# qiutang98/chord

Hardware: AMD Instinct MI355X
Metric: Gtri/s into 4K 64-bit visbuffer (higher is better)
Workload: dtype f32+u64; 1 GPU; street_4k_hzb; scene_triangles_lod0=2799616, objects=352, hzb=True, cull=flat, parallelism=single

## Files before the change

### chord_amd/csrc/chordvis_abi.cpp

```cpp

#include "device_layer.h"

#include <algorithm>
#include <cmath>
#include <cstddef>
#include <cstdio>
#include <cstring>

using namespace chord;

namespace chord {

int fail(ChordCtx* ctx, int code, const char* what, hipError_t e)
{
    if (ctx) {
        char buf[512];
        if (e != hipSuccess) std::snprintf(buf, sizeof(buf), "%s: %s (%d)", what, hipGetErrorString(e), (int)e);
        else std::snprintf(buf, sizeof(buf), "%s", what);
        ctx->lastError = buf;
    }
    return code;
}

}
// ... 1360 lines not shown
    CHORD_HIP(c, hipMemcpy(c->hzb[slot].minTexels, hostMin, sizeof(uint16_t) * c->hzb[slot].desc.totalTexels, hipMemcpyHostToDevice));
    c->hzb[slot].valid = true;
    c->hzb[slot].uploaded = true;
    c->historySlot = slot;
    return CHORDVIS_OK;
}

int chordvis_set_debug(ChordCtx* c, uint32_t flags)
{
    if (c) c->orderAge = c->orderAge1 = 0xFFFFFFFFu;

    if (!c) return CHORDVIS_E_INVALID;
    if (!RASTER_PROFILE && (flags & CHORD_DEBUG_PROFILE_BITS))
        return fail(c, CHORDVIS_E_INVALID, "set_debug: the phase clocks (bits 16, 512) need a library built with -DRASTER_PROFILE=1 (chord_amd/build.py --tag prof -DRASTER_PROFILE=1)");
    if (!RASTER_ABLATION && (flags & CHORD_DEBUG_ABLATION_BITS))
        return fail(c, CHORDVIS_E_INVALID, "set_debug: the ablation switches need a library built with -DRASTER_ABLATION=1 (chord_amd/build.py --tag abl -DRASTER_ABLATION=1)");
    c->debugFlags = flags;
    if (c->depthCtx) c->depthCtx->debugFlags = flags;
    return CHORDVIS_OK;
}

int chordvis_debug_tile_profile(ChordCtx* c, int pass, uint64_t* hostTicks, uint32_t* hostCounts, uint32_t capacity)
{
    if (!c || pass < 0 || pass > 1 || !hostTicks || !hostCounts || capacity < c->tilesX * c->tilesY) return fail(c, CHORDVIS_E_INVALID, "debug_tile_profile: bad arguments");
    CHORD_HIP(c, hipStreamSynchronize(c->stream));
    const size_t n = (size_t)c->tilesX * c->tilesY;
    CHORD_HIP(c, hipMemcpy(hostTicks, c->dTileClocks + (size_t)pass * CHORD_MAX_TILES, n * 8, hipMemcpyDeviceToHost));
    CHORD_HIP(c, hipMemcpy2D(hostCounts, 4, c->dFrameState->tileCount + (size_t)pass * c->tilesX * c->tilesY * CHORD_TILECOUNT_STRIDE, 4 * CHORD_TILECOUNT_STRIDE, 4, n, hipMemcpyDeviceToHost));
    if (capacity >= 9 * n)
        CHORD_HIP(c, hipMemcpy(hostTicks + n, c->dTileClocks + (size_t)2 * CHORD_MAX_TILES + (size_t)pass * CHORD_MAX_TILES * 8, n * 64, hipMemcpyDeviceToHost));
    return CHORDVIS_OK;
}

int chordvis_debug_graph_frames(ChordCtx* c, uint32_t pairs, float* msPerFrameStream, float* msPerFrameGraph)
{
    if (!c || !pairs || !msPerFrameStream || !msPerFrameGraph) return fail(c, CHORDVIS_E_INVALID, "debug_graph_frames: bad arguments");
    if (!c->ownStream) return fail(c, CHORDVIS_E_INVALID, "debug_graph_frames: needs a context-owned (capturable) stream");
    int rc;
    struct KeepOff { ChordCtx* c; uint32_t keep; ~KeepOff() { c->orderKeepFrames = keep; c->orderAge = c->orderAge1 = 0xFFFFFFFFu; } } keepOff{c, c->orderKeepFrames};
    c->orderKeepFrames = 0u;
    for (int i = 0; i < 4; i++) if ((rc = chordvis_render_frame(c))) return rc;
    hipEvent_t e0, e1;
    CHORD_HIP(c, hipEventCreate(&e0)); CHORD_HIP(c, hipEventCreate(&e1));
    CHORD_HIP(c, hipStreamSynchronize(c->stream));
    CHORD_HIP(c, hipEventRecord(e0, c->stream));
    for (uint32_t i = 0; i < 2 * pairs; i++) if ((rc = chordvis_render_frame(c))) return rc;
    CHORD_HIP(c, hipEventRecord(e1, c->stream));
    CHORD_HIP(c, hipEventSynchronize(e1));
    float ms = 0;
    CHORD_HIP(c, hipEventElapsedTime(&ms, e0, e1));
    *msPerFrameStream = ms / (2.0f * pairs);
    hipGraph_t graph; hipGraphExec_t exec;
    CHORD_HIP(c, hipStreamBeginCapture(c->stream, hipStreamCaptureModeRelaxed));
    rc = chordvis_render_frame(c);
    if (!rc) rc = chordvis_render_frame(c);
    hipError_t ce = hipStreamEndCapture(c->stream, &graph);
    if (rc) return rc;
    CHORD_HIP(c, ce);
    CHORD_HIP(c, hipGraphInstantiate(&exec, graph, nullptr, nullptr, 0));
    for (int i = 0; i < 4; i++) CHORD_HIP(c, hipGraphLaunch(exec, c->stream));
    CHORD_HIP(c, hipStreamSynchronize(c->stream));
    CHORD_HIP(c, hipEventRecord(e0, c->stream));
    for (uint32_t i = 0; i < pairs; i++) CHORD_HIP(c, hipGraphLaunch(exec, c->stream));
    CHORD_HIP(c, hipEventRecord(e1, c->stream));
    CHORD_HIP(c, hipEventSynchronize(e1));
    CHORD_HIP(c, hipEventElapsedTime(&ms, e0, e1));
// ... 143 lines not shown
```

### chord_amd/csrc/device_layer.h

```cpp
#pragma once

#include <hip/hip_runtime.h>
#include <cstddef>

#include <string>
#include <vector>

#include "chordvis.h"

#ifndef RASTER_PROFILE
#define RASTER_PROFILE 0
#endif
#ifndef RASTER_ABLATION
#define RASTER_ABLATION 0
#endif
#define CHORD_DEBUG_PROFILE_BITS (16u | 512u)
#define CHORD_DEBUG_ABLATION_BITS (1u | 2u | 32u | 64u | 128u | 256u | 1024u | 2048u | 4096u | 8192u | 16384u | 1048576u | 2097152u)

namespace chord {


struct DPrim {
    float    posMin[3]; uint32_t meshletBase;
    float    posMax[3]; uint32_t groupBase;
// ... 325 lines not shown
    uint32_t* dTileBins = nullptr;
    uint32_t* dBinPool = nullptr;
    unsigned long long* dBinChunkTab = nullptr;
    uint32_t binPoolChunks = 0;
    uint32_t binMaxChunks = CHORD_BIN_MAX_CHUNKS_DEFAULT;
    uint64_t limitRecords = 64ull << 20;
    uint32_t limitPoolChunks = 32768;
    uint32_t rasterSerial = 0;
    bool inFrame = false;
    uint32_t binCap = 0, tilesX = 0, tilesY = 0;
    chord::ClipTri* dClipTris = nullptr;
    uint32_t clipTriCap = 0;
    bool resolveFrame = false;
    bool resolveStale = false;
    uint32_t* dTileMarker = nullptr;
    uint32_t* dShadingTiles = nullptr;
    uint32_t* dTileOrder = nullptr;
    uint32_t* dTileOrderKeep = nullptr;
    uint32_t orderAge = 0xFFFFFFFFu;
    uint32_t* dTileOrderKeep1 = nullptr;
    uint32_t orderAge1 = 0xFFFFFFFFu;
    uint32_t orderFlip[2] = {0u, 0u};
    uint32_t orderKeepFrames = 1u;
    unsigned long long* dTileSlabs = nullptr;
    uint32_t tileItemCap = 0;
    uint32_t* dLargeList = nullptr;
    uint32_t largeCap = 0;
    chord::DeviceCounters* dCounters = nullptr;
    bool pendingClear = false;
    bool depthOnly = false, depthClamp = false;
    float depthBiasConst = 0.0f, depthBiasSlope = 0.0f;

    uint64_t launchCount = 0;
    uint64_t frameLaunchBase = 0;
    uint32_t lastFrameLaunches = 0;
    int timers = 0;
    std::vector<hipEvent_t> evPool;
    std::vector<int> stampTags;
    uint32_t framesStamped = 0;
    uint32_t timerPeriod = 1;
    uint32_t frameIndex = 0;
    bool stampThisFrame = false;
    uint32_t rasterCalls = 0;
    bool shouldStage1 = false;
    chord::CmdList lastRejected;
    bool hzbTailInCull = false;
    bool fuseCullFrame = false;
    const chord::HzbBuffers* fuseCullHzb = nullptr;
    bool fusedCullDone = false;
    uint32_t cullSerial = 0;
    unsigned long long* dCullLookback = nullptr;
    uint32_t debugFlags = 0;
    unsigned long long* dTileClocks = nullptr;
};

#define CHORD_LAUNCH(ctx, ...) do { (ctx)->launchCount++; hipLaunchKernelGGL(__VA_ARGS__); } while (0)

namespace chord {

int fail(ChordCtx* ctx, int code, const char* what, hipError_t e = hipSuccess);
int alloc_scene_work_buffers(ChordCtx* c);

#define CHORD_HIP(ctx, call)                                                         \
    do {                                                                             \
        hipError_t e_ = (call);                                                      \
        if (e_ != hipSuccess) return ::chord::fail((ctx), CHORDVIS_E_HIP, #call, e_); \
// ... 32 lines not shown
```

### chord_amd/csrc/kernels_raster.hip

```cpp

#include "device_layer.h"
#include "device_math.h"

#include <algorithm>
#include <cstdlib>
#include <cstring>
#include <type_traits>

namespace chord {

#define GUARD_BAND 1024.0f
#define LDS_VERTS 256
#define TILE CHORD_TILE
#define TILE_SHIFT CHORD_TILE_SHIFT
#define TPITCH (TILE + 1)
#define SMALL_AREA 256
#define TC_STRIDE CHORD_TILECOUNT_STRIDE
#define TC_BLOCKS 1u
#define TC_TICKET 2u
#ifndef CHORD_MASKED_FUSED
#define CHORD_MASKED_FUSED 1
#endif
#define TC_MASKED 3u

// ... 15 lines not shown
    unsigned long long* binChunkTab; uint32_t binStamp; uint32_t binMaxChunks;
    unsigned long long* blockPool; uint32_t blockCap;
    uint32_t blockForce;
    ClipTri* clipTris; uint32_t clipTriCap; uint32_t pass;
    uint32_t* largeList; uint32_t largeCap;
    uint32_t binInSetup;
    DeviceCounters* counters;
    uint2* tileOrder;
    unsigned long long* tileSlabs;
    uint32_t hzbFused;
    ChordHZBDesc hzbDesc;
    uint16_t* hzbMinA;
    uint16_t* hzbMinB; uint16_t* hzbMaxB;
    uint16_t* hzbExA;
    uint16_t* hzbExB;
    uint32_t* tileRange;
    unsigned long long* tileClocks;
    unsigned long long* tilePhase;
    uint32_t depthOnly, depthClamp;
    float biasConst, biasSlope;
    uint32_t clearTiles;
    uint32_t* binHint;
    uint32_t* countHint;
    uint32_t slotHot;
    uint32_t* hotTiles;
    uint32_t tileSlots;
    uint32_t tileSplitMin, tileSliceLen;
    uint2* tileOrderNext;
    uint32_t orderAll;
    uint32_t orderKept;
    uint32_t* heavyHint;
    uint32_t* tileTouched;
    uint32_t debug;
};
#define ABL(p, flag) (RASTER_ABLATION && ((p).debug & (flag)) != 0u)
#define DBG_NO_PIXELS   1u
#define DBG_NO_BIN      2u
#define DBG_TILE_CLOCKS 16u
#define DBG_NO_OUT      128u
#define DBG_NO_HZB      256u
#define DBG_SETUP_CLOCKS 512u
#define DBG_NO_VIS_STORE 1024u
#define DBG_NO_SPLIT    2048u
#define DBG_NO_TINY     32u
#define DBG_TILE_EXIT   64u
#define DBG_NO_ENTRY    8192u
#define DBG_NO_BATCH    16384u
#define DBG_NO_UNITS    4096u
#define DBG_SKIP_LIGHT  1048576u
#define DBG_SKIP_HEAVY  2097152u

template <typename T>
__device__ __forceinline__ T scalar_load(const T* ptr)
{
    return *reinterpret_cast<const __attribute__((address_space(4))) T*>(reinterpret_cast<uintptr_t>(ptr));
}
__device__ __forceinline__ const RasterParams* kernel_args()
{
    unsigned long long kp = (unsigned long long)__builtin_amdgcn_kernarg_segment_ptr();
    asm volatile("" : "+s"(kp));
    return reinterpret_cast<const RasterParams*>(kp);
}

__device__ __forceinline__ uint32_t mbcnt64(unsigned long long m) { return __builtin_amdgcn_mbcnt_hi((uint32_t)(m >> 32), __builtin_amdgcn_mbcnt_lo((uint32_t)m, 0u)); }
__device__ __forceinline__ int32_t bcast(int32_t v, int src) { return __builtin_amdgcn_readlane(v, src); }
__device__ __forceinline__ uint32_t bcast(uint32_t v, int src) { return (uint32_t)__builtin_amdgcn_readlane((int)v, src); }
// ... 1400 lines not shown
#undef SPHASE
}

__device__ __forceinline__ bool launch_is_dense(const RasterParams& p, uint32_t count)
{
    const unsigned long long pixels = (unsigned long long)p.Wi * (unsigned long long)p.Hi / (p.shard.ranks > 1u ? p.shard.ranks : 1u);
    return p.blockCap != 0u && p.leftCmds != nullptr && (p.blockForce != 0u || (unsigned long long)count * 16ull >= pixels);
}

#ifndef SETUP_MIN_WAVES
#define SETUP_MIN_WAVES 5
#endif
#ifndef BLOCKS_MIN_WAVES
#define BLOCKS_MIN_WAVES 6
#endif
#ifndef SETUP_MASKED_WAVES
#define SETUP_MASKED_WAVES 4
#endif
template <bool MASKED>
__global__ __launch_bounds__(256, MASKED ? SETUP_MASKED_WAVES : SETUP_MIN_WAVES) void raster_setup_kernel(RasterParams p)
{
    __shared__ __attribute__((aligned(16))) float sVert[6][4][LDS_VERTS];
    __shared__ uint32_t sClip[4][1 + CLIP_RANGES];
    const uint32_t c0 = __builtin_amdgcn_readfirstlane(min(blockIdx.x * 4u + (threadIdx.x >> 6), p.cmdCap - 1u));
    const uint32_t* __restrict__ cw = reinterpret_cast<const uint32_t*>(p.cmds + c0);
    const uint32_t f0 = scalar_load(cw), f1 = scalar_load(cw + 1), f2 = scalar_load(cw + 2);
    uint32_t count = *p.count;
    const ChordDrawCmd* cmds = p.cmds;
    bool firstValid = true;
    if (launch_is_dense(p, count)) { count = *p.leftCount; cmds = p.leftCmds; firstValid = false; }
    raster_setup_body<MASKED>(p, cmds, count, sVert, sClip[threadIdx.x >> 6], f0, f1, f2, firstValid);
}

template <bool HOT>
__global__ __launch_bounds__(256, BLOCKS_MIN_WAVES) void raster_setup_blocks_kernel(RasterParams p)
{
    __shared__ float sVert[6][4][BLOCKS_LDS_VERTS];
    __shared__ int32_t sSnap[2][4][BLOCKS_LDS_VERTS];
    __shared__ unsigned long long sWin[4][WIN * WIN];
    __shared__ SlotCache sSlots[HOT ? 4 : 1];
    const uint32_t count = *p.count;
    if (!launch_is_dense(p, count)) return;
    raster_setup_blocks_body<HOT>(p, count, sVert, sSnap, sWin, sSlots);
}

__device__ void raster_clip_part(const RasterParams& p, uint32_t block, uint32_t blocks)
{
    __shared__ float4 sPoly[2 * CLIP_MAXV * CLIP_THREADS];
    __shared__ float sPU[2 * CLIP_MAXV * CLIP_THREADS], sPV[2 * CLIP_MAXV * CLIP_THREADS];
    __shared__ int32_t sPX[CLIP_MAXV * CLIP_THREADS], sPY[CLIP_MAXV * CLIP_THREADS];
    __shared__ float sPD[CLIP_MAXV * CLIP_THREADS];
    if (threadIdx.x >= CLIP_THREADS) return;
    const ClipLds<CLIP_THREADS> L = {sPoly, sPU, sPV, sPX, sPY, sPD, threadIdx.x};
    const uint32_t n = min(p.counters->clipTriCount[p.pass], p.clipTriCap);
    const uint32_t listShard = block % CHORD_LIST_SHARDS;
    for (uint32_t k = block * CLIP_THREADS + threadIdx.x; k < n; k += blocks * CLIP_THREADS) {
        clip_entry<true>(p, L, p.clipTris[k], listShard);
    }
}

#define CLIP_BLOCKS 64u
__device__ void raster_bin_large_part(const RasterParams& p, uint32_t block, uint32_t blocks)
{
    const uint32_t lane = threadIdx.x & 63u, wave = threadIdx.x >> 6;
    __shared__ uint32_t sStart[CHORD_LIST_SHARDS + 1];
    if (threadIdx.x < 64u) {
// ... 1453 lines not shown
    }
    p.orderKept = 0u;
    p.heavyHint = nullptr;
    static const bool directOn = [] { const char* e = getenv("CHORDVIS_TILE_DIRECT"); return !e || atoi(e) != 0; }();
    const bool laterOk = c->inFrame && !clearTiles && p.hzbFused && !c->depthOnly && CHORD_MASKED_FUSED && c->dBinHint && !(c->debugFlags & ~(DBG_NO_BLOCKS | DBG_FORCE_BLOCKS | DBG_FORCE_HOT | 524288u));
    if (laterOk) p.heavyHint = c->dBinHint + 4 + pass;
    if (TILE_DIRECT && directOn && laterOk) {
        const uint32_t heavySeen = c->hBinHint[4 + pass], lightSeen = c->hBinHint[6 + pass];
        if (lightSeen != 0u && (heavySeen == 0u || (int32_t)(lightSeen - heavySeen) > 0)) {
            p.orderKept = 2u;
        }
    }
    static const int touchedEnv = [] { const char* e = getenv("CHORDVIS_TILE_TOUCHED"); return e ? atoi(e) : 1; }();
    p.tileTouched = nullptr;
    if (p.orderKept == 2u && touchedEnv != 0 && c->shard.ranks <= 1 && tiles <= 64u * 64u) {
        p.tileTouched = c->dFrameState->tileTouched + (size_t)pass * (CHORD_MAX_TILES / 32u);
        if (!c->inFrame || c->rasterCalls >= 2) LR_HIP(hipMemsetAsync(p.tileTouched, 0, sizeof(uint32_t) * ((tiles + 31u) / 32u), c->stream));
    }
    uint32_t blocks = (in.capacity + 3u) / 4u;
#ifndef SETUP_GRID_MULT
#define SETUP_GRID_MULT 1u
#endif
    const uint32_t maxBlocks = (uint32_t)c->numCUs * SETUP_MIN_WAVES * SETUP_GRID_MULT;
    if (blocks > maxBlocks) blocks = maxBlocks;
    if (blocks < 1) blocks = 1;
    const bool sh = c->shard.ranks > 1;
    stamp(c, S_HZBCULL);
    if (blocksWorthLaunching) {
        const uint32_t bb = std::max(1u, std::min((in.capacity + 3u) / 4u, (uint32_t)c->numCUs * BLOCKS_MIN_WAVES));
        const bool hot = (c->hBinHint && c->hBinHint[pass] >= SLOT_HOT) || (c->debugFlags & DBG_FORCE_HOT);
        if (hot) CHORD_LAUNCH(c, raster_setup_blocks_kernel<true>, dim3(bb), dim3(256), 0, c->stream, p);
        else     CHORD_LAUNCH(c, raster_setup_blocks_kernel<false>, dim3(bb), dim3(256), 0, c->stream, p);
    }
    if (c->anyMasked) CHORD_LAUNCH(c, raster_setup_kernel<true>, dim3(blocks), dim3(256), 0, c->stream, p);
    else              CHORD_LAUNCH(c, raster_setup_kernel<false>, dim3(blocks), dim3(256), 0, c->stream, p);
    stamp(c, S_R_CLUSTER);
    if (!p.binInSetup) CHORD_LAUNCH(c, raster_clip_and_bin_large_kernel, dim3(CLIP_BLOCKS + (uint32_t)c->numCUs * 4u), dim3(256), 0, c->stream, p);
    bool makeOrder = p.orderKept != 2u;
    p.orderAll = 0u; p.tileOrderNext = nullptr;
    static const bool keepLaterOn = [] { const char* e = getenv("CHORDVIS_TILE_KEEP_LATER"); return !e || atoi(e) != 0; }();
    static const bool nextOn = [] { const char* e = getenv("CHORDVIS_TILE_NEXT"); return !e || atoi(e) != 0; }();
    const bool keepOk = TILE_ORDER_KEEP && c->orderKeepFrames && CHORD_MASKED_FUSED && c->inFrame && !c->depthOnly && !(c->debugFlags & ~524288u);
    int slot = -1;
    if (keepOk && clearTiles && pass == 0u && c->dTileOrderKeep) slot = 0;
    else if (keepOk && keepLaterOn && laterOk && pass == 1u && c->dTileOrderKeep1) slot = 1;
    if (slot >= 0) {
        uint32_t& age = slot ? c->orderAge1 : c->orderAge;
        uint2* buf = reinterpret_cast<uint2*>(slot ? c->dTileOrderKeep1 : c->dTileOrderKeep);
        const size_t half = (size_t)1 + c->tileItemCap;
        p.orderAll = slot ? 1u : 0u;
        if (nextOn && p.orderKept == 2u) {
            age = 0xFFFFFFFFu; p.orderAll = 0u;
        } else if (nextOn) {
            uint32_t& flip = c->orderFlip[slot];
            p.tileOrder = buf + flip * half; p.tileOrderNext = buf + (flip ^ 1u) * half;
            if (age != 0xFFFFFFFFu) { p.orderKept = 1u; makeOrder = false; }
            age = 0u; flip ^= 1u;
        } else if (p.orderKept != 2u) {
            p.tileOrder = buf;
            if (age < c->orderKeepFrames) { age++; p.orderKept = 1u; makeOrder = false; }
            else age = 0u;
        } else p.orderAll = 0u;
    }
    if (makeOrder) CHORD_LAUNCH(c, raster_tile_order_kernel, dim3(1), dim3(1024), 0, c->stream, p);
#if !CHORD_MASKED_FUSED
    if (c->anyMasked) {
        const uint32_t items = tiles;
        if (c->depthClamp && !sh) CHORD_LAUNCH(c, (raster_masked_tile_kernel<false, true>), dim3(items), dim3(TB), 0, c->stream, p);
// ... 29 lines not shown
```

### chord_amd/lib.py

```python
import ctypes as C
import os

import numpy as np

from . import records as R

_HERE = os.path.dirname(os.path.abspath(__file__))
LIB_PATH = os.environ.get("CHORDVIS_LIB") or os.path.join(_HERE, "_build", "libchordvis.so")

OK, E_INVALID, E_HIP, E_NO_DEVICE, E_CAPACITY, E_COMM = 0, -1, -2, -3, -4, -5


class ChordvisError(RuntimeError):
    pass


class CountAndCmd(C.Structure):
    _fields_ = [("count", C.c_void_p), ("cmds", C.c_void_p), ("capacity", C.c_uint32)]


class Limits(C.Structure):
    _fields_ = [("maxTriangleRecords", C.c_uint64), ("binPoolChunks", C.c_uint32), ("binMaxChunksPerTile", C.c_uint32)]


# ... 163 lines not shown
        "chordvis_comm_unique_id": (i32, [vp]),
        "chordvis_comm_init_rank": (i32, [vp, u32, u32, vp]),
        "chordvis_comm_destroy": (i32, [vp]),
        "chordvis_comm_set_pipelined": (i32, [vp, vp]),
        "chordvis_comm_info": (i32, [vp, P(i32), P(u32), vp, u32]),
        "chordvis_create_group": (i32, [u32, P(i32), P(vp)]),
        "chordvis_destroy_group": (i32, [vp]),
        "chordvis_group_size": (u32, [vp]),
        "chordvis_group_ctx": (vp, [vp, u32]),
        "chordvis_group_last_error": (C.c_char_p, [vp]),
        "chordvis_group_set_limits": (i32, [vp, P(Limits)]),
        "chordvis_group_upload_scene": (i32, [vp, P(R.SceneDesc)]),
        "chordvis_group_allocate_gbuffer": (i32, [vp, u32, u32]),
        "chordvis_group_rebalance": (i32, [vp, vp]),
        "chordvis_group_update_objects": (i32, [vp, vp, u32]),
        "chordvis_group_set_view": (i32, [vp, vp, vp, u32]),
        "chordvis_group_render_frame": (i32, [vp]),
        "chordvis_group_sync": (i32, [vp]),
        "chordvis_group_enqueue_ms": (i32, [vp, vp, u32]),
        "chordvis_group_set_pipelined": (i32, [vp, i32]),
        "chordvis_allocate_depth_views": (i32, [vp, u32, u32]),
        "chordvis_set_instance_views": (i32, [vp, vp, u32]),
        "chordvis_instance_culling_view": (i32, [vp, u32, P(CountAndCmd)]),
        "chordvis_hzb_culling_generic": (i32, [vp, P(HZB), C.c_float, u32, i32, CountAndCmd, P(CountAndCmd)]),
        "chordvis_render_mesh_depth": (i32, [vp, u32, i32, C.c_float, C.c_float, CountAndCmd, P(DepthTarget)]),
        "chordvis_build_hzb_from_depth": (i32, [vp, P(DepthTarget), P(HZB)]),
        "chordvis_readback_depth": (i32, [vp, P(DepthTarget), vp]),
        "chordvis_depth_view_stats": (i32, [vp, P(Stats)]),
        "chordvis_render_shadow": (i32, [vp, vp, vp, vp, u32, i32, vp, vp, P(u32)]),
        "chordvis_enable_timers": (i32, [vp, i32]),
        "chordvis_stats": (i32, [vp, P(Stats)]),
        "chordvis_set_debug": (i32, [vp, u32]),
        "chordvis_debug_tile_profile": (i32, [vp, i32, vp, vp, u32]),
        "chordvis_debug_setup_profile": (i32, [vp, i32, vp, P(u32)]),
        "chordvis_debug_read": (i32, [vp, i32, C.c_uint64, C.c_uint64, vp]),
        "chordvis_debug_slab_nonzero": (i32, [vp, P(C.c_uint64)]),
        "chordvis_debug_graph_frames": (i32, [vp, u32, P(C.c_float), P(C.c_float)]),
    }
    missing = []
    for name, (res, args) in protos.items():
        try:
            fn = getattr(lib, name)
        except AttributeError:
            missing.append(name)
            continue
        fn.restype, fn.argtypes = res, args
    if missing and os.environ.get("CHORDVIS_AB_OLD_LIB") == "1":
        missing = []
    if missing:
        raise ChordvisError("libchordvis.so lacks symbols declared in include/chordvis.h: %s" % ", ".join(missing))
    return lib, sorted(protos)


lib, EXPORTED = _load()



def hzb_desc(width, height):
    d = R.HZBDesc()
    rc = lib.chordvis_hzb_desc(width, height, C.byref(d))
    if rc != OK:
        raise ChordvisError("chordvis_hzb_desc(%d, %d) -> %d" % (width, height, rc))
    return d


def make_views(camera, last_view=None):
# ... 81 lines not shown
```

### include/chordvis.h

```cpp
#ifndef CHORDVIS_H
#define CHORDVIS_H

#include "chordvis_types.h"

#ifdef __cplusplus
extern "C" {
#endif
#if defined(__GNUC__)
#pragma GCC visibility push(default)
#endif

#define CHORDVIS_OK              0
#define CHORDVIS_E_INVALID      -1
#define CHORDVIS_E_HIP          -2
#define CHORDVIS_E_NO_DEVICE    -3
#define CHORDVIS_E_CAPACITY     -4
#define CHORDVIS_E_COMM         -5

typedef struct ChordCtx ChordCtx;

typedef struct ChordCountAndCmd {
    uint32_t*     count;
    ChordDrawCmd* cmds;
    uint32_t      capacity;
// ... 235 lines not shown
typedef struct ChordResolveTargets {
    float*    barycentrics;
    float*    baryDdx;
    float*    baryDdy;
    float*    uv;
    float*    uvGrad;
    float*    positionRS;
    float*    motionVector;
    uint32_t* debugRGBA8;
} ChordResolveTargets;
int chordvis_resolve_attributes(ChordCtx* ctx, ChordCountAndCmd drawedMeshletCmd, const ChordResolveDesc* desc,
                                const ChordResolveTargets* targets);
void* chordvis_stream(ChordCtx* ctx);


int chordvis_readback_visibility(ChordCtx* ctx, uint64_t* hostWords );
int chordvis_readback_previous_visibility(ChordCtx* ctx, uint64_t* hostWords);
int chordvis_readback_cmds(ChordCtx* ctx, ChordCountAndCmd handle, ChordDrawCmd* hostCmds, uint32_t cap, uint32_t* outCount);
int chordvis_readback_hzb(ChordCtx* ctx, const ChordHZB* hzb, uint16_t* hostMin, uint16_t* hostMax, uint32_t hostValidRange[2]);
int chordvis_readback_tile_marker(ChordCtx* ctx, const ChordTileMarker* marker, uint32_t* host);
int chordvis_readback_shading_tiles(ChordCtx* ctx, const ChordShadingTiles* tiles, uint32_t* hostTiles, uint32_t hostCapacity,
                                    uint32_t* hostCount, uint32_t hostDispatchArgs[4]);
int chordvis_upload_history_hzb(ChordCtx* ctx, const uint16_t* hostMin);

int chordvis_enable_timers(ChordCtx* ctx, int mode);
int chordvis_stats(ChordCtx* ctx, ChordStats* out);
int chordvis_set_debug(ChordCtx* ctx, uint32_t flags);
int chordvis_debug_fill_cull_exchange(ChordCtx* ctx);
int chordvis_debug_read(ChordCtx* ctx, int which, uint64_t offset, uint64_t bytes, void* host);
int chordvis_debug_slab_nonzero(ChordCtx* ctx, uint64_t* count);
int chordvis_debug_graph_frames(ChordCtx* ctx, uint32_t pairs, float* msPerFrameStream, float* msPerFrameGraph);
int chordvis_debug_setup_profile(ChordCtx* ctx, int pass, uint64_t hostTicks[5], uint32_t* waves);
int chordvis_debug_tile_profile(ChordCtx* ctx, int pass, uint64_t* hostTicks, uint32_t* hostCounts, uint32_t capacity);

#if defined(__GNUC__)
#pragma GCC visibility pop
#endif
#ifdef __cplusplus
}
#endif
#endif
```

Measured before the change: 3.390 Gtri/s.

## Add one-meshlet-per-block wide setup kernel with LDS tile-hash binning

Adds a setup kernel that gives each 256-thread block one meshlet at a time, with a persistent grid stride, when the cluster count is small. Triangle-to-tile bin entries are grouped in an LDS hash table so each tile gets a single global atomicAdd per block. Large triangles are spread across all threads through a prefix scan. The aim is more parallelism and fewer global atomics when there are few clusters, at the cost of extra barriers and LDS hashing. A branch in the kernel falls back to the old body when the count exceeds wideMax.

```diff
diff --git a/chord_amd/csrc/chordvis_abi.cpp b/chord_amd/csrc/chordvis_abi.cpp
--- a/chord_amd/csrc/chordvis_abi.cpp
+++ b/chord_amd/csrc/chordvis_abi.cpp
@@ -1416,6 +1416,13 @@
     return CHORDVIS_OK;
 }
 
+int chordvis_debug_setup_kernels(ChordCtx* c, uint32_t wide[2])
+{
+    if (!c || !wide) return fail(c, CHORDVIS_E_INVALID, "debug_setup_kernels: bad arguments");
+    wide[0] = c->setupWide[0]; wide[1] = c->setupWide[1];
+    return CHORDVIS_OK;
+}
+
 int chordvis_debug_graph_frames(ChordCtx* c, uint32_t pairs, float* msPerFrameStream, float* msPerFrameGraph)
 {
     if (!c || !pairs || !msPerFrameStream || !msPerFrameGraph) return fail(c, CHORDVIS_E_INVALID, "debug_graph_frames: bad arguments");
diff --git a/chord_amd/csrc/device_layer.h b/chord_amd/csrc/device_layer.h
--- a/chord_amd/csrc/device_layer.h
+++ b/chord_amd/csrc/device_layer.h
@@ -381,6 +381,7 @@
     float depthBiasConst = 0.0f, depthBiasSlope = 0.0f;
 
     uint64_t launchCount = 0;
+    uint32_t setupWide[2] = {0, 0};
     uint64_t frameLaunchBase = 0;
     uint32_t lastFrameLaunches = 0;
     int timers = 0;
diff --git a/chord_amd/csrc/kernels_raster.hip b/chord_amd/csrc/kernels_raster.hip
--- a/chord_amd/csrc/kernels_raster.hip
+++ b/chord_amd/csrc/kernels_raster.hip
@@ -71,6 +71,7 @@
     uint32_t* heavyHint;
     uint32_t* tileTouched;
     uint32_t debug;
+    uint32_t wideMax;
 };
 #define ABL(p, flag) (RASTER_ABLATION && ((p).debug & (flag)) != 0u)
 #define DBG_NO_PIXELS   1u
@@ -1537,6 +1538,302 @@
     raster_setup_body<MASKED>(p, cmds, count, sVert, sClip[threadIdx.x >> 6], f0, f1, f2, firstValid);
 }
 
+#define WIDE_HASH 1024u
+#define WIDE_EMPTY 0xFFFFFFFFu
+#ifndef SETUP_WIDE_WAVES
+#define SETUP_WIDE_WAVES 4
+#endif
+template <bool MASKED>
+__global__ __launch_bounds__(256, SETUP_WIDE_WAVES) void raster_setup_wide_kernel(RasterParams p)
+{
+    __shared__ __attribute__((aligned(16))) float sVert[6][4][LDS_VERTS];
+    __shared__ uint32_t sClipW[4][1 + CLIP_RANGES];
+    float* const sBuf = &sVert[0][0][0];
+    float (*const sV)[LDS_VERTS] = reinterpret_cast<float (*)[LDS_VERTS]>(sBuf);
+    uint32_t* const sKey = reinterpret_cast<uint32_t*>(sBuf + 12u * LDS_VERTS);
+    uint32_t* const sCnt = sKey + WIDE_HASH;
+    uint32_t* const sIncl = sCnt + WIDE_HASH;
+    uint32_t (*const sWave)[4] = reinterpret_cast<uint32_t (*)[4]>(sIncl + 128);
+    uint32_t* const sBase = sIncl + 128 + 16;
+    static_assert(12u * LDS_VERTS + 2u * WIDE_HASH + 128u + 16u + 3u <= 6u * 4u * LDS_VERTS, "the wide form's arrays fit sVert");
+    uint32_t* const sClip = sClipW[0];
+    const uint32_t tid = threadIdx.x, lane = tid & 63u, wave = tid >> 6;
+    const uint32_t c0 = __builtin_amdgcn_readfirstlane(min(blockIdx.x, p.cmdCap - 1u));
+    const uint32_t* __restrict__ cw0 = reinterpret_cast<const uint32_t*>(p.cmds + c0);
+    const uint32_t f0 = scalar_load(cw0), f1 = scalar_load(cw0 + 1), f2 = scalar_load(cw0 + 2);
+    uint32_t count = *p.count;
+    const ChordDrawCmd* cmds = p.cmds;
+    bool firstValid = true;
+    if (launch_is_dense(p, count)) { count = *p.leftCount; cmds = p.leftCmds; firstValid = false; }
+    count = __builtin_amdgcn_readfirstlane(count);
+    if (count > p.wideMax) {
+        raster_setup_body<MASKED>(p, cmds, count, sVert, sClipW[wave], 0u, 0u, 0u, false);
+        return;
+    }
+    if (blockIdx.x >= count) return;
+
+    auto header_of = [&](uint32_t objectId, uint32_t meshletId, uint32_t slot) -> SetupHeader {
+        SetupHeader h;
+        h.objectId = objectId; h.meshletId = meshletId; h.slot = slot;
+        const DMeshlet* __restrict__ mm = &p.meshlets[meshletId];
+        const uint32_t vt = scalar_load(&mm->vertexTriangleCount);
+        h.V = vt & 0xFFu; h.T = (vt >> 8) & 0xFFu;
+        h.dataOffset = scalar_load(&mm->dataOffset);
+        h.vertexBase = scalar_load(&mm->vertexBase);
+        h.matFlags = scalar_load(&p.objStatic[objectId].matFlags);
+        if (CHORD_MATFLAG_ALPHA(h.matFlags) >= CHORD_ALPHA_BLEND) h.T = 0u;
+        return h;
+    };
+    auto load_header = [&](uint32_t i) -> SetupHeader {
+        const uint32_t k = __builtin_amdgcn_readfirstlane(min(i, count - 1u));
+        const uint32_t* __restrict__ cw = reinterpret_cast<const uint32_t*>(cmds + k);
+        return header_of(scalar_load(cw), scalar_load(cw + 1), scalar_load(cw + 2));
+    };
+    float* lX = sV[0]; float* lY = sV[1]; float* lW = sV[2]; float* lU = sV[3]; float* lV = sV[4]; float* lD = sV[5];
+    const LargeLds LL = {{sV[6], sV[7], sV[8], sV[9], sV[10]}};
+    const uint32_t listShard = blockIdx.x % CHORD_LIST_SHARDS;
+    const uint32_t t = wave * 32u + lane;
+    SetupHeader hdr = firstValid ? header_of(f0, f1, f2) : load_header(blockIdx.x);
+    if (tid == 0u) sClip[0] = 0u;
+    for (uint32_t c = blockIdx.x; c < count; c += gridDim.x) {
+        const SetupHeader hdrN = load_header(c + gridDim.x);
+        const uint32_t V = hdr.V, T = min(hdr.T, 128u), dataOffset = hdr.dataOffset, vertexBase = hdr.vertexBase;
+        const bool twoSided = (hdr.matFlags & CHORD_MATFLAG_TWO_SIDED) != 0u || p.depthOnly != 0u;
+        const bool masked = MASKED && CHORD_MATFLAG_ALPHA(hdr.matFlags) == CHORD_ALPHA_MASK;
+        const uint32_t* __restrict__ md = p.meshletData;
+        const bool hasTri = lane < 32u && t < T;
+        const uint32_t triWord = hasTri ? md[dataOffset + V + t] : 0u;
+        Mat4 mvp;
+        {
+            const float* __restrict__ mv = p.objFrame[hdr.objectId].mvp;
+#pragma unroll
+            for (int r = 0; r < 4; r++)
+#pragma unroll
+                for (int cc = 0; cc < 4; cc++) mvp.r[r][cc] = scalar_load(mv + r * 4 + cc);
+        }
+        for (uint32_t h = tid; h < WIDE_HASH; h += 256u) { sKey[h] = WIDE_EMPTY; sCnt[h] = 0u; }
+        if (tid < V) {
+            const float* __restrict__ pp = p.positions + (size_t)((md[dataOffset + tid] + vertexBase) * 3u);
+            const f4 h = mul_mv(mvp, pp[0], pp[1], pp[2], 1.0f);
+            const float aw = fabsf(h.w);
+            lX[tid] = h.x; lY[tid] = h.y; lW[tid] = h.w;
+            lU[tid] = h.x / aw * 0.5f + 0.5f;
+            lV[tid] = h.y / aw * -0.5f + 0.5f;
+            const bool fast = p.depthClamp ? in_fast_volume_xy(h) : in_fast_volume(h);
+            lD[tid] = fast ? h.z / h.w : __builtin_nanf("");
+        }
+        float uv[6] = {0.0f, 0.0f, 0.0f, 0.0f, 0.0f, 0.0f};
+        if (MASKED && masked && hasTri && p.texcoords != nullptr) {
+#pragma unroll
+            for (int i = 0; i < 3; i++) {
+                const size_t vi = (size_t)(md[dataOffset + ((triWord >> (8 * i)) & 0xFFu)] + vertexBase) * 2;
+                uv[2 * i] = p.texcoords[vi]; uv[2 * i + 1] = p.texcoords[vi + 1];
+            }
+        }
+        __syncthreads();
+        int kind = K_NONE;
+        TriSetup ts;
+        ts.px0 = ts.py0 = ts.px1 = ts.py1 = 0;
+        float d[3] = {0.0f, 0.0f, 0.0f};
+        if (hasTri) {
+            const uint32_t i0 = triWord & 0xFFu, i1 = (triWord >> 8) & 0xFFu, i2 = (triWord >> 16) & 0xFFu;
+            const float x0 = lX[i0], y0 = lY[i0], w0 = lW[i0];
+            const float x1 = lX[i1], y1 = lY[i1], w1 = lW[i1];
+            const float x2 = lX[i2], y2 = lY[i2], w2 = lW[i2];
+            bool culled = false;
+            if (!twoSided) {
+                const float det = (x0 * (y1 * w2 - w1 * y2) - y0 * (x1 * w2 - w1 * x2)) + w0 * (x1 * y2 - y1 * x2);
+                culled = det <= 0.0f;
+            }
+            culled = culled || (w0 <= 0.0f && w1 <= 0.0f && w2 <= 0.0f);
+            const float u0 = lU[i0], v0 = lV[i0], u1 = lU[i1], v1 = lV[i1], u2 = lU[i2], v2 = lV[i2];
+            const float maxU = fmaxf(u0, fmaxf(u1, u2)), maxV = fmaxf(v0, fmaxf(v1, v2));
+            const float minU = fminf(u0, fminf(u1, u2)), minV = fminf(v0, fminf(v1, v2));
+            culled = culled || ((minU >= 1.0f || minV >= 1.0f) || (maxU <= 0.0f || maxV <= 0.0f));
+            culled = culled || (rintf(minU * p.W) == rintf(maxU * p.W) || rintf(minV * p.H) == rintf(maxV * p.H));
+            if (!culled) {
+                d[0] = lD[i0]; d[1] = lD[i1]; d[2] = lD[i2];
+                ts.payload = p.depthOnly ? 0u : encode_triangle_instance(t, hdr.slot);
+                if (d[0] != d[0] || d[1] != d[1] || d[2] != d[2]) {
+                    kind = K_CLIP;
+                } else {
+                    ts.X[0] = (int32_t)rintf((u0 * p.W) * 256.0f); ts.Y[0] = (int32_t)rintf((v0 * p.H) * 256.0f);
+                    ts.X[1] = (int32_t)rintf((u1 * p.W) * 256.0f); ts.Y[1] = (int32_t)rintf((v1 * p.H) * 256.0f);
+                    ts.X[2] = (int32_t)rintf((u2 * p.W) * 256.0f); ts.Y[2] = (int32_t)rintf((v2 * p.H) * 256.0f);
+                    if (tri_setup(ts, twoSided, p.Wi, p.Hi) && owns_rect(p.shard, ts.px0, ts.py0, ts.px1, ts.py1)) {
+                        kind = K_EMIT;
+                        if (p.biasConst != 0.0f || p.biasSlope != 0.0f) { const float o = depth_bias(ts, d, p.biasConst, p.biasSlope); d[0] += o; d[1] += o; d[2] += o; }
+                    }
+                }
+            }
+        }
+        if (ABL(p, DBG_NO_BIN)) kind = K_NONE;
+        const unsigned long long lt = (1ull << lane) - 1ull;
+        const bool cp = kind == K_EMIT && !masked && fits_compact(ts);
+        const bool lg = kind == K_EMIT && touches_many_tiles(ts);
+        const unsigned long long cm = __ballot(kind == K_CLIP), ec = __ballot(cp), ew = __ballot(kind == K_EMIT && !cp), lm = __ballot(lg);
+        if (lane == 0u) {
+            sWave[wave][0] = (uint32_t)__popcll(cm); sWave[wave][1] = (uint32_t)__popcll(ec);
+            sWave[wave][2] = (uint32_t)__popcll(ew); sWave[wave][3] = (uint32_t)__popcll(lm);
+        }
+        uint32_t tileR[4], hR[4], rankR[4], has = 0u;
+#pragma unroll
+        for (int r = 0; r < 4; r++) {
+            const int32_t tx0 = ts.px0 >> TILE_SHIFT, tx1 = ts.px1 >> TILE_SHIFT, ty0 = ts.py0 >> TILE_SHIFT, ty1 = ts.py1 >> TILE_SHIFT;
+            const int32_t tx = (r & 1) ? tx1 : tx0, ty = (r & 2) ? ty1 : ty0;
+            bool in = kind == K_EMIT && !lg && !((r & 1) && tx1 == tx0) && !((r & 2) && ty1 == ty0);
+            if (in) in = owns_tile(p.shard, tx, ty);
+            tileR[r] = in ? __umul24((uint32_t)ty, p.tilesX) + (uint32_t)tx : 0u;
+            hR[r] = 0u; rankR[r] = 0u;
+            if (in) {
+                has |= 1u << r;
+                uint32_t h = tileR[r] & (WIDE_HASH - 1u);
+                for (;;) {
+                    const uint32_t o = atomicCAS(&sKey[h], WIDE_EMPTY, tileR[r]);
+                    if (o == WIDE_EMPTY || o == tileR[r]) break;
+                    h = (h + 1u) & (WIDE_HASH - 1u);
+                }
+                hR[r] = h;
+                rankR[r] = atomicAdd(&sCnt[h], 1u);
+            }
+        }
+        __syncthreads();
+        const uint32_t nClip = sWave[0][0] + sWave[1][0] + sWave[2][0] + sWave[3][0];
+        const uint32_t nLg = sWave[0][3] + sWave[1][3] + sWave[2][3] + sWave[3][3];
+        {
+            uint32_t n[4], key[4], base[4];
+#pragma unroll
+            for (int i = 0; i < 4; i++) { n[i] = sCnt[tid + 256u * i]; key[i] = sKey[tid + 256u * i]; }
+            uint32_t cbase = 0u, ebaseC = 0u, ebaseW = 0u;
+            if (tid == 0u) {
+                const uint32_t nEc = sWave[0][1] + sWave[1][1] + sWave[2][1] + sWave[3][1];
+                const uint32_t nEw = sWave[0][2] + sWave[1][2] + sWave[2][2] + sWave[3][2];
+                if (nClip) cbase = atomicAdd(&p.counters->clipTriCount[p.pass], nClip);
+                if (nEc) ebaseC = atomicAdd(&p.counters->triCountC[listShard * CHORD_SHARD_STRIDE], nEc);
+                if (nEw) ebaseW = atomicAdd(&p.counters->triCount[listShard * CHORD_SHARD_STRIDE], nEw * (masked ? 1u + CHORD_MASK_EXT_SLOTS : 1u));
+                if (nLg) atomicAdd(&p.counters->largeCount[p.pass][listShard * CHORD_SHARD_STRIDE], nLg);
+            }
+#pragma unroll
+            for (int i = 0; i < 4; i++) base[i] = n[i] ? atomicAdd(&p.tileCount[(size_t)key[i] * TC_STRIDE], n[i]) : 0u;
+            if (MASKED && masked) {
+#pragma unroll
+                for (int i = 0; i < 4; i++) if (n[i]) p.tileCount[(size_t)key[i] * TC_STRIDE + TC_MASKED] = 1u;
+            }
+#pragma unroll
+            for (int i = 0; i < 4; i++) if (n[i]) sCnt[tid + 256u * i] = base[i];
+            if (tid == 0u) {
+                sBase[0] = cbase; sBase[1] = ebaseC; sBase[2] = ebaseW;
+                if (nClip) {
+                    const uint32_t r = sClip[0];
+                    if (r < CLIP_RANGES) { sClip[1u + r] = cbase | (nClip - 1u) << 25; sClip[0] = r + 1u; } else atomicOr(&p.counters->overflow, 2u);
+                }
+            }
+        }
+        __syncthreads();
+        {
+            uint32_t offClip = 0u, offC = 0u, offW = 0u;
+            for (uint32_t w = 0; w < wave; w++) { offClip += sWave[w][0]; offC += sWave[w][1]; offW += sWave[w][2]; }
+            const uint32_t wSlots = masked ? 1u + CHORD_MASK_EXT_SLOTS : 1u;
+            uint32_t slotR[4];
+#pragma unroll
+            for (int r = 0; r < 4; r++) slotR[r] = (has & (1u << r)) ? sCnt[hR[r]] + rankR[r] : 0u;
+            if (kind == K_CLIP) {
+                const uint32_t k = sBase[0] + offClip + (uint32_t)__popcll(cm & lt);
+                if (k < p.clipTriCap) { ClipTri ct; ct.objectId = hdr.objectId; ct.meshletId = hdr.meshletId; ct.slot = hdr.slot; ct.tri = t; p.clipTris[k] = ct; }
+                else atomicOr(&p.counters->overflow, 2u);
+            }
+            uint32_t gi = 0u;
+            bool ok = false;
+            if (cp) {
+                const uint32_t li = sBase[1] + offC + (uint32_t)__popcll(ec & lt);
+                if (li < p.triCapC) { gi = listShard * p.triCapC + li; write_record_c(&p.trisC[gi], ts, d); ok = true; }
+                else atomicOr(&p.counters->overflow, 1u);
+            } else if (kind == K_EMIT) {
+                const uint32_t li = sBase[2] + wSlots * (offW + (uint32_t)__popcll(ew & lt));
+                if (li + wSlots <= p.triCap) {
+                    gi = listShard * p.triCap + li; write_record(&p.tris[gi], ts, d, twoSided, masked);
+                    if (MASKED && masked) setup_emit_mask_ext(p, &p.tris[gi + 1u], triWord, uv, lW, CHORD_MATFLAG_MATERIAL(hdr.matFlags), ts.area);
+                    gi |= (MASKED && masked) ? CHORD_REC_MASKED : CHORD_REC_WIDE; ok = true;
+                } else atomicOr(&p.counters->overflow, 1u);
+            }
+#pragma unroll
+            for (int r = 0; r < 4; r++) if (has & (1u << r)) bin_alloc(p, tileR[r], slotR[r]);
+            if (ok) {
+#pragma unroll
+                for (int r = 0; r < 4; r++) if (has & (1u << r)) bin_put(p, tileR[r], slotR[r], gi);
+            }
+            if (nLg) {
+                uint32_t nt = 0u;
+                if (lg && ok) {
+                    large_put(LL, t, ts);
+                    LL.at(LG_GI, t) = gi;
+                    nt = large_tiles(LL.at(LG_BX, t), LL.at(LG_BY, t));
+                }
+                if (lane < 32u) sIncl[t] = nt;
+            }
+        }
+        if (nLg) {
+            __syncthreads();
+            if (wave == 0u) {
+                const uint32_t a = sIncl[2u * lane], b = sIncl[2u * lane + 1u];
+                uint32_t incl = a + b;
+#pragma unroll
+                for (int dd = 1; dd < 64; dd <<= 1) { const uint32_t nb = (uint32_t)__shfl_up((int)incl, dd, 64); if (lane >= (uint32_t)dd) incl += nb; }
+                sIncl[2u * lane] = incl - b; sIncl[2u * lane + 1u] = incl;
+            }
+            __syncthreads();
+            const uint32_t total = sIncl[127];
+            for (uint32_t j = tid; j < total; j += 256u) {
+                uint32_t k = 0u;
+#pragma unroll
+                for (uint32_t st = 64u; st > 0u; st >>= 1) if (sIncl[k + st - 1u] <= j) k += st;
+                const uint32_t tt = j - (k ? sIncl[k - 1u] : 0u);
+                TriSetup lr;
+#pragma unroll
+                for (int i = 0; i < 3; i++) { lr.X[i] = (int32_t)LL.at(LG_X0 + i, k); lr.Y[i] = (int32_t)LL.at(LG_Y0 + i, k); }
+                lr.s = (int32_t)LL.at(LG_S, k);
+                const uint32_t bx = LL.at(LG_BX, k), by = LL.at(LG_BY, k), lgi = LL.at(LG_GI, k);
+                lr.px0 = (int32_t)(bx & 0xFFFFu); lr.px1 = (int32_t)(bx >> 16); lr.py0 = (int32_t)(by & 0xFFFFu); lr.py1 = (int32_t)(by >> 16);
+                const int32_t tx0 = lr.px0 >> TILE_SHIFT, ty0 = lr.py0 >> TILE_SHIFT;
+                const uint32_t tw = (uint32_t)((lr.px1 >> TILE_SHIFT) - tx0 + 1);
+                const int32_t tx = tx0 + (int32_t)(tt % tw), ty = ty0 + (int32_t)(tt / tw);
+                const int32_t rx0 = max(lr.px0, tx << TILE_SHIFT), rx1 = min(lr.px1, (tx << TILE_SHIFT) + TILE - 1);
+                const int32_t ry0 = max(lr.py0, ty << TILE_SHIFT), ry1 = min(lr.py1, (ty << TILE_SHIFT) + TILE - 1);
+                const int ea[3] = {1, 2, 0}, eb[3] = {2, 0, 1};
+                bool hit = owns_tile(p.shard, tx, ty);
+#pragma unroll
+                for (int i = 0; i < 3; i++) {
+                    const int64_t dxe = (int64_t)(lr.X[eb[i]] - lr.X[ea[i]]), dye = (int64_t)(lr.Y[eb[i]] - lr.Y[ea[i]]);
+                    const int64_t a = -(int64_t)lr.s * dye, b = (int64_t)lr.s * dxe;
+                    const int64_t bias = (a > 0 || (a == 0 && b > 0)) ? 0 : -1;
+                    const int64_t cx = (int64_t)(a > 0 ? rx1 : rx0) * 256 + 128, cy = (int64_t)(b > 0 ? ry1 : ry0) * 256 + 128;
+                    hit = hit && !((int64_t)lr.s * (dxe * (cy - lr.Y[ea[i]]) - dye * (cx - lr.X[ea[i]])) + bias < 0);
+                }
+                if (!hit) continue;
+                const uint32_t tile = (uint32_t)ty * p.tilesX + (uint32_t)tx;
+                bin_store(p, tile, atomicAdd(&p.tileCount[(size_t)tile * TC_STRIDE], 1u), lgi);
+                if ((lgi & 0xE0000000u) == CHORD_REC_MASKED) p.tileCount[(size_t)tile * TC_STRIDE + TC_MASKED] = 1u;
+            }
+        }
+        __syncthreads();
+        hdr = hdrN;
+    }
+    __syncthreads();
+    if (const uint32_t ranges = sClip[0]) {
+        float* a = sV[3u * wave]; float* b = sV[3u * wave + 1u]; float* cc = sV[3u * wave + 2u];
+        const ClipLds<CLIP_SETUP_LANES> L = {reinterpret_cast<float4*>(a), b, b + 2u * CLIP_MAXV * CLIP_SETUP_LANES,
+                                             reinterpret_cast<int32_t*>(cc), reinterpret_cast<int32_t*>(cc) + CLIP_MAXV * CLIP_SETUP_LANES,
+                                             cc + 2u * CLIP_MAXV * CLIP_SETUP_LANES, lane};
+        for (uint32_t i = 0; i < ranges; i++) {
+            const uint32_t w = sClip[1u + i], base = w & 0x1FFFFFFu, n = (w >> 25) + 1u;
+            for (uint32_t k0 = 0; k0 < n; k0 += 4u * CLIP_SETUP_LANES) {
+                const uint32_t k = k0 + wave * CLIP_SETUP_LANES + lane;
+                if (lane < CLIP_SETUP_LANES && k < n && base + k < p.clipTriCap) clip_entry<MASKED>(p, L, p.clipTris[base + k], listShard);
+            }
+        }
+    }
+}
+
 template <bool HOT>
 __global__ __launch_bounds__(256, BLOCKS_MIN_WAVES) void raster_setup_blocks_kernel(RasterParams p)
 {
@@ -3056,8 +3353,16 @@
         if (hot) CHORD_LAUNCH(c, raster_setup_blocks_kernel<true>, dim3(bb), dim3(256), 0, c->stream, p);
         else     CHORD_LAUNCH(c, raster_setup_blocks_kernel<false>, dim3(bb), dim3(256), 0, c->stream, p);
     }
-    if (c->anyMasked) CHORD_LAUNCH(c, raster_setup_kernel<true>, dim3(blocks), dim3(256), 0, c->stream, p);
-    else              CHORD_LAUNCH(c, raster_setup_kernel<false>, dim3(blocks), dim3(256), 0, c->stream, p);
+    static const int setupWide = [] { const char* e = getenv("CHORDVIS_SETUP_WIDE"); return e ? atoi(e) : 1; }();
+    p.wideMax = setupWide > 1 ? (uint32_t)setupWide : TILE_DIRECT_MAX_CLUSTERS;
+    c->setupWide[pass] = 0u;
+    if (setupWide != 0 && p.orderKept == 2u && p.binInSetup && !blocksWorthLaunching && !sh) {
+        const uint32_t wideBlocks = std::max(1u, std::min(std::max(in.capacity, 1u), (uint32_t)c->numCUs * SETUP_WIDE_WAVES));
+        if (c->anyMasked) CHORD_LAUNCH(c, raster_setup_wide_kernel<true>, dim3(wideBlocks), dim3(256), 0, c->stream, p);
+        else              CHORD_LAUNCH(c, raster_setup_wide_kernel<false>, dim3(wideBlocks), dim3(256), 0, c->stream, p);
+        c->setupWide[pass] = 1u;
+    } else if (c->anyMasked) CHORD_LAUNCH(c, raster_setup_kernel<true>, dim3(blocks), dim3(256), 0, c->stream, p);
+    else                     CHORD_LAUNCH(c, raster_setup_kernel<false>, dim3(blocks), dim3(256), 0, c->stream, p);
     stamp(c, S_R_CLUSTER);
     if (!p.binInSetup) CHORD_LAUNCH(c, raster_clip_and_bin_large_kernel, dim3(CLIP_BLOCKS + (uint32_t)c->numCUs * 4u), dim3(256), 0, c->stream, p);
     bool makeOrder = p.orderKept != 2u;
diff --git a/chord_amd/lib.py b/chord_amd/lib.py
--- a/chord_amd/lib.py
+++ b/chord_amd/lib.py
@@ -219,6 +219,7 @@
         "chordvis_stats": (i32, [vp, P(Stats)]),
         "chordvis_set_debug": (i32, [vp, u32]),
         "chordvis_debug_tile_profile": (i32, [vp, i32, vp, vp, u32]),
+        "chordvis_debug_setup_kernels": (i32, [vp, P(u32)]),
         "chordvis_debug_setup_profile": (i32, [vp, i32, vp, P(u32)]),
         "chordvis_debug_read": (i32, [vp, i32, C.c_uint64, C.c_uint64, vp]),
         "chordvis_debug_slab_nonzero": (i32, [vp, P(C.c_uint64)]),
diff --git a/include/chordvis.h b/include/chordvis.h
--- a/include/chordvis.h
+++ b/include/chordvis.h
@@ -291,6 +291,7 @@
 int chordvis_debug_graph_frames(ChordCtx* ctx, uint32_t pairs, float* msPerFrameStream, float* msPerFrameGraph);
 int chordvis_debug_setup_profile(ChordCtx* ctx, int pass, uint64_t hostTicks[5], uint32_t* waves);
 int chordvis_debug_tile_profile(ChordCtx* ctx, int pass, uint64_t* hostTicks, uint32_t* hostCounts, uint32_t capacity);
+int chordvis_debug_setup_kernels(ChordCtx* ctx, uint32_t wide[2]);
 
 #if defined(__GNUC__)
 #pragma GCC visibility pop
```

Result: faster. 3.471 Gtri/s, median of 6 (+2.4%).
